# wustl-cig/FLAIR

Measured on AMD Instinct MI355X. Metric: restored frames/sec at 256x256, 16-frame clip, 250-step DDIM, higher is better.
Workload: dtype bf16

## Files before the change

### flair_amd/_lib.py

```python
import ctypes
import os

import torch

_HERE = os.path.dirname(os.path.abspath(__file__))
LIB_PATH = os.path.join(_HERE, "libflair_hip.so")

FLAIR_F32, FLAIR_BF16 = 0, 1
ACT_NONE, ACT_RELU, ACT_LRELU01, ACT_SILU, ACT_DCN_OFFSETS, ACT_LRELU02, ACT_GELU = 0, 1, 2, 3, 4, 5, 6


class FlairHipUnavailable(RuntimeError):
    pass


class FlairHipError(RuntimeError):
    pass


class ConvParams(ctypes.Structure):
    _fields_ = [("dtype", ctypes.c_int), ("T", ctypes.c_int), ("H", ctypes.c_int),
                ("W", ctypes.c_int), ("KT", ctypes.c_int), ("KH", ctypes.c_int),
                ("KW", ctypes.c_int), ("Cout", ctypes.c_int), ("nseg", ctypes.c_int),
                ("seg_c", ctypes.c_int * 4), ("seg_ld", ctypes.c_int * 4),
                ("y_ld", ctypes.c_int), ("res_ld", ctypes.c_int * 2), ("act", ctypes.c_int),
                ("out_scale", ctypes.c_float), ("frame_bias_ld", ctypes.c_int), ("stride", ctypes.c_int),
                ("act_param", ctypes.c_float), ("act_period", ctypes.c_int), ("asym_pad", ctypes.c_int),
                ("reflect_pad", ctypes.c_int)]


_lib = None


def lib():
    global _lib
    if _lib is None:
        global LIB_PATH
        if os.environ.get("FLAIR_HIP_LIB"):
            LIB_PATH = os.environ["FLAIR_HIP_LIB"]
        if not os.path.exists(LIB_PATH):
            raise FlairHipUnavailable(
                f"{LIB_PATH} not found: build it with `python -c 'import __graft_entry__ as g; "
                f"g.build()'` (or `make -C flair_amd/csrc`). The HIP library is required; "
# ... 43 lines not shown
```

### flair_amd/csrc/chain.hip

```cpp
#include <type_traits>

#include "common.h"

namespace {

struct ChainArgs {
    const void* x[4];
    int segC[4], segLd[4], nseg;
    unsigned segBytes[4];
    const void* wA; const float* biasA; int actA; int CinA; unsigned wABytes;
    const void* wB; const float* biasB; int actB; int CoutB; unsigned wBBytes;
    const void* res0; const void* res1; int res0Ld, res1Ld;
    float outScale;
    float actParam; int actPeriod;
    void* y; int yLd;
    int T, H, W;
};

template <typename E> struct MmaC;
template <> struct MmaC<bf16_t> {
    static constexpr int BKE = 32;
    static __device__ __forceinline__ int chunk(int i, int half) { return 2 * i + half; }
    static __device__ __forceinline__ void run(const uint4 (&a)[2], const uint4 (&b)[2], f32x16& acc) {
        acc = __builtin_amdgcn_mfma_f32_32x32x16_bf16(__builtin_bit_cast(bf16x8, a[0]),
                                                      __builtin_bit_cast(bf16x8, b[0]), acc, 0, 0, 0);
        acc = __builtin_amdgcn_mfma_f32_32x32x16_bf16(__builtin_bit_cast(bf16x8, a[1]),
// ... 357 lines not shown
                        }
                    }
                }
            }
        }
        if (batch + 1 < nBatch) {
            write_w(0);
            __syncthreads();
        }
    }
}

struct ResArgs {
    const void* x; int xLd; unsigned xBytes;
    const void* w; unsigned wBytes;
    const float* bias;
    int Cout, act;
    float actParam; int actPeriod;
    float outScale;
    void* y; int yLd;
    int T, H, W;
};

template <int ACT, int NW>
__global__ __launch_bounds__(64 * NW, NW / 4) void conv_resident_kernel(ResArgs a) {
    static_assert(NW == 8, "eight waves of one row");
    prefetch_kernargs<sizeof(ResArgs)>();
    using E = bf16_t;
    constexpr int RPW = 8 / NW;
    constexpr int HWP = 34, HROWS = 10 * HWP, HINSTR = (HROWS + 15) / 16, HBYTES = HINSTR * 1024;
// ... 26 lines not shown
            const int R = k * 16 + lrow;
            const int hr = R / HWP, c = R - hr * HWP;
            const int hh = h0 - 1 + hr, ww = w0 - 1 + c;
            const bool ok = R < HROWS && (unsigned)hh < (unsigned)a.H && (unsigned)ww < (unsigned)a.W;
            const unsigned voff = ok ? (unsigned)(hh * a.W + ww) * ldB + (unsigned)(ch * 64) + (unsigned)((lchunk ^ ((c >> 2) & 3)) << 4) : FLAIR_OOB;
            dma16(xdesc, voff, (unsigned)(ch * HBYTES + k * 1024));
        }
    };
    issue_halo(0);
    unsigned wlane[NWS];
    int wco[NWS];
#pragma unroll
    for (int i = 0; i < NWS; ++i) {
        const int id = (wave * NWS + i) % WINSTR;
        const int row = id * 16 + lrow, tap9 = row >> 6, co = row & 63;
        wlane[i] = (unsigned)((co * 9 + tap9) * 64) * 2u + (unsigned)((lchunk ^ ((co >> 2) & 3)) << 4);
        wco[i] = co;
    }
    auto issue_w = [&](int s_) {
        const int blk = s_ >> 1, ch = s_ & 1;
        const unsigned base = (unsigned)(blk * 64 * 9 * 64) * 2u + (unsigned)(ch * 64);
        const unsigned dst = (unsigned)(RING + (s_ % NRING) * SLOT);
#pragma unroll
        for (int i = 0; i < NWS; ++i) {
            const int id = (wave * NWS + i) % WINSTR;
            dma16(wdesc, blk * 64 + wco[i] < a.Cout ? base + wlane[i] : FLAIR_OOB, dst + (unsigned)(id * 1024));
        }
    };
    auto issue_w_one = [&](int s_, int i) {
        const int blk = s_ >> 1, ch = s_ & 1;
        const unsigned base = (unsigned)(blk * 64 * 9 * 64) * 2u + (unsigned)(ch * 64);
        const int id = (wave * NWS + i) % WINSTR;
        dma16(wdesc, blk * 64 + wco[i] < a.Cout ? base + wlane[i] : FLAIR_OOB, (unsigned)(RING + (s_ % NRING) * SLOT + id * 1024));
    };
    issue_w(0);
    issue_halo(1);
    if (nS > 1) issue_w(1);

    unsigned aoff[2], boff[3][2];
#pragma unroll
    for (int ks = 0; ks < 2; ++ks) {
        aoff[ks] = (unsigned)(lr * 64 + (((2 * ks + lh) ^ ((lr >> 2) & 3)) << 4));
#pragma unroll
        for (int kw = 0; kw < 3; ++kw)
            boff[kw][ks] = (unsigned)((RPW * wave * HWP + kw + lr) * 64 + (((2 * ks + lh) ^ (((kw + lr) >> 2) & 3)) << 4));
    }
// ... 125 lines not shown
        block(blk, acc0, acc1);
        if (blk + 1 < nBlk) block(blk + 1, acc1, acc0);
    }
    if (nBlk & 1) {
#pragma unroll
        for (int g = 0; g < 4 * RPW; ++g) epi_piece(acc0, nBlk - 1, g);
    } else {
#pragma unroll
        for (int g = 0; g < 4 * RPW; ++g) epi_piece(acc1, nBlk - 1, g);
    }
}

int launch_resident(const ChainArgs& c, hipStream_t s) {
    ResArgs a;
    a.x = c.x[0]; a.xLd = c.segLd[0]; a.xBytes = c.segBytes[0];
    a.w = c.wB; a.wBytes = c.wBBytes; a.bias = c.biasB; a.Cout = c.CoutB; a.act = c.actB;
    a.actParam = c.actParam; a.actPeriod = c.actPeriod; a.outScale = c.outScale;
    a.y = c.y; a.yLd = c.yLd; a.T = c.T; a.H = c.H; a.W = c.W;
    constexpr size_t lds = 2 * 22 * 1024 + 3 * 36 * 1024 + 2048;
    const int grid = a.T * (a.H / 8) * (a.W / 32);
    auto go = [&](auto tag) -> int {
        constexpr int ACT = decltype(tag)::value;
        static LdsAttrOnce attr;
        const hipError_t e = flair_max_lds_once(attr, reinterpret_cast<const void*>(&conv_resident_kernel<ACT, 8>));
        FLAIR_CHECK(e == hipSuccess, "flair_conv_chain: hipFuncSetAttribute: %s", hipGetErrorString(e));
        hipLaunchKernelGGL((conv_resident_kernel<ACT, 8>), dim3(grid), dim3(64 * 8), lds, s, a);
        FLAIR_LAUNCH_CHECK();
        return FLAIR_OK;
    };
    if (a.act == FLAIR_ACT_DCN_OFFSETS) return go(std::integral_constant<int, 1>{});
    if (a.act == FLAIR_ACT_SILU) return go(std::integral_constant<int, 2>{});
// ... 367 lines not shown
                "flair_conv_chain: res1 stride/alignment");
    a.res0 = res0; a.res1 = res1; a.res0Ld = p->res_ld[0]; a.res1Ld = p->res_ld[1];
    a.outScale = p->out_scale;
    a.actParam = p->act_param; a.actPeriod = p->act_period;
    FLAIR_CHECK(p->actA != FLAIR_ACT_DCN_OFFSETS && (p->actB != FLAIR_ACT_DCN_OFFSETS ||
                                                       (p->act_period > 0 && p->act_period % 24 == 0)),
                "flair_conv_chain: FLAIR_ACT_DCN_OFFSETS is a stage-B activation with act_period = 3 * deform_groups");
    {
        auto plain = [](int c) { return c == FLAIR_ACT_NONE || c == FLAIR_ACT_RELU || c == FLAIR_ACT_LRELU01 || c == FLAIR_ACT_SILU; };
        FLAIR_CHECK(plain(p->actA) && (plain(p->actB) || p->actB == FLAIR_ACT_DCN_OFFSETS),
                    "flair_conv_chain: activation codes (%d, %d) unsupported: NONE / RELU / LRELU01 / SILU (+ DCN_OFFSETS for stage B)",
                    p->actA, p->actB);
    }
    a.y = y; a.yLd = p->y_ld;
    a.T = p->T; a.H = p->H; a.W = p->W;
    if (!hasA && p->dtype == FLAIR_BF16 && p->C == 64 && p->W % 32 == 0 && p->H % 8 == 0 && !res0 && !res1 &&
        (p->y_ld * 2) % 16 == 0 && p->CoutB % 8 == 0 &&
        (unsigned long long)p->H * p->W * p->y_ld * 2 < 0x40000000ull)
        return launch_resident(a, stream);
    {
        auto lin = [](int c) { return c == FLAIR_ACT_NONE || c == FLAIR_ACT_RELU || c == FLAIR_ACT_LRELU01; };
        if (hasA && p->dtype
 == FLAIR_BF16 && p->C == 64 && p->nseg == 1 && cin == 64 && p->CoutB == 64 && p->W % 32 == 0 &&
            p->H % 8 == 0 && lin(p->actA) && lin(p->actB) && (unsigned long long)p->H * p->W * p->y_ld * 2 < 0x40000000ull &&
            (!res0 || (unsigned long long)p->H * p->W * p->res_ld[0] * 2 < 0x40000000ull) &&
            (!res1 || (unsigned long long)p->H * p->W * p->res_ld[1] * 2 < 0x40000000ull))
            return launch_pair(a, stream);
    }
    if (p->dtype == FLAIR_BF16)
        return hasA ? dispatch_chain<bf16_t, true>(a, p->C, stream) : dispatch_chain<bf16_t, false>(a, p->C, stream);
// ... 3 lines not shown
```

### flair_amd/csrc/conv.hip

```cpp
#include <type_traits>

#include "common.h"

namespace {

struct ConvArgs {
    const void* x[4];
    int segC[4];
    int segLd[4];
    int nseg;
    const void* w;
    const float* bias;
    const void* res0;
    const void* res1;
    int res0Ld, res1Ld;
    void* y;
    int yLd;
    int T, H, W;
    int KT, KH, KW;
    int Cout, CinTot;
    int act;
    float outScale;
    long P;
    int nPixTiles, nCoTiles;
    int tFast;
    unsigned segBytes[4];
    unsigned wBytes;
    float* part;
    int splitK;
    const float* fbias;
    int fbiasLd;
    int stride;
    int tapShift;
    int reflect;
    float actParam;
    int actPeriod;
    int Hin, Win;
    int esz;
};

template <typename E> struct Mma;

template <> struct Mma<bf16_t> {
    static constexpr int BKE = 32;
    static __device__ __forceinline__ int chunk(int i, int half) { return 2 * i + half; }
    static __device__ __forceinline__ void run(const uint4 (&a)[2], const uint4 (&b)[2], f32x16& acc) {
        acc = __builtin_amdgcn_mfma_f32_32x32x16_bf16(__builtin_bit_cast(bf16x8, a[0]),
                                                      __builtin_bit_cast(bf16x8, b[0]), acc, 0, 0, 0);
        acc = __builtin_amdgcn_mfma_f32_32x32x16_bf16(__builtin_bit_cast(bf16x8, a[1]),
                                                      __builtin_bit_cast(bf16x8, b[1]), acc, 0, 0, 0);
    }
    static __device__ __forceinline__ void run1(const uint4& a, const uint4& b, f32x16& acc) {
        acc = __builtin_amdgcn_mfma_f32_32x32x16_bf16(__builtin_bit_cast(bf16x8, a), __builtin_bit_cast(bf16x8, b),
                                                      acc, 0, 0, 0);
// ... 1178 lines not shown
    constexpr int HINSTR = 22, HIMG = HINSTR * 1024, WINSTR = 36, SLOT = WINSTR * 1024;
    constexpr int HR = 3, WR = 2;
    constexpr int RING = HR * HIMG, BIAS = RING + WR * SLOT;
    constexpr int NH = (HINSTR + NW - 1) / NW, NWS = (WINSTR + NW - 1) / NW;
    extern __shared__ __attribute__((aligned(16))) char smem[];
    const int tid = threadIdx.x, lane = tid & 63;
    const int wave = __builtin_amdgcn_readfirstlane(tid >> 6);
    const int lr = lane & 31, lh = lane >> 5;
    const int lrow = lane >> 2, lchunk = lane & 3;
    const int tilesW = a.W / 32, perFrame = tilesW * (a.H / 8);
    const int bid = xcd_remap(blockIdx.x, gridDim.x);
    const int t = bid / perFrame, tile = bid - t * perFrame;
    const int h0 = (tile / tilesW) * 8, w0 = (tile % tilesW) * 32;
    const int nS = a.CinTot / 32;

    const u32x4_t wdesc = make_desc(a.w, a.wBytes);
    const u32x4_t bdesc = make_desc(a.bias, a.bias ? (unsigned)a.Cout * 4u : 0u);
    dma16(bdesc, (unsigned)(lane * 16), (unsigned)BIAS);
    unsigned hpix[NH], hpiece[NH];
#pragma unroll
    for (int i = 0; i < NH; ++i) {
        const int k = (wave * NH + i) % HINSTR;
        const int R = k * 16 + lrow;
        const int hr = R / HWP, c = R - hr * HWP;
        const int hh = h0 - 1 + hr, ww = w0 - 1 + c;
        const bool ok = R < 10 * HWP && (unsigned)hh < (unsigned)a.H && (unsigned)ww < (unsigned)a.W;
        hpix[i] = ok ? (unsigned)(hh * a.W + ww) : 0xffffffffu;
        hpiece[i] = (unsigned)((lchunk ^ ((c >> 2) & 3)) << 4);
    }
    unsigned wlane[NWS];
#pragma unroll
    for (int i = 0; i < NWS; ++i) {
        const int id = (wave * NWS + i) % WINSTR;
        const int row = id * 16 + lrow, tap9 = row >> 6, co = row & 63;
        wlane[i] = co < a.Cout ? (unsigned)((co * 9 + tap9) * a.CinTot) * 2u + (unsigned)((lchunk ^ ((co >> 2) & 3)) << 4) : FLAIR_OOB;
    }
    int hseg = 0, hcb = 0;
    auto issue_halo = [&](int slot) {
        const unsigned ld = (unsigned)a.segLd[hseg] * 2u;
        const u32x4_t xdesc = make_desc(reinterpret_cast<const char*>(a.x[hseg]) + (size_t)t * a.H * a.W * ld, a.segBytes[hseg]);
        const unsigned cofs = (unsigned)(hcb * 64);
#pragma unroll
        for (int i = 0; i < NH; ++i) {
            const int k = (wave * NH + i) % HINSTR;
            dma16(xdesc, hpix[i] == 0xffffffffu ? FLAIR_OOB : hpix[i] * ld + cofs + hpiece[i], (unsigned)(slot * HIMG + k * 1024));
        }
        if (++hcb * 32 >= a.segC[hseg]) {
            hcb = 0;
            ++hseg;
        }
    };
    auto issue_w = [&](int s_) {
#pragma unroll
        for (int i = 0; i < NWS; ++i) {
            const int id = (wave * NWS + i) % WINSTR;
            dma16(wdesc, wlane[i] == FLAIR_OOB ? FLAIR_OOB : wlane[i] + (unsigned)(s_ * 64), (unsigned)(RING + (s_ % WR) * SLOT + id * 1024));
        }
    };
    issue_halo(0);
    issue_w(0);
    if (nS > 1) {
        issue_halo(1);
        issue_w(1);
    }
    if (nS > 2) issue_halo(2);

    unsigned aoff[2], boff[3][2];
#pragma unroll
    for (int ks = 0; ks < 2; ++ks) {
        aoff[ks] = (unsigned)(lr * 64 + (((2 * ks + lh) ^ ((lr >> 2) & 3)) << 4));
#pragma unroll
// ... 431 lines not shown
        return 5;
    }
    const long tiles128 = (long)cdiv(a.P, 128) * cdiv(a.Cout, 128);
    if (a.Cout > 64 && tiles128 >= 512) return 0;
    if (a.Cout >= 128 && a.P >= 1024 && tiles128 <= 64 && (long)a.KT * a.KH * a.KW * a.CinTot >= 2304) return 0;
    const long tiles64x128 = (long)cdiv(a.P, 128) * cdiv(a.Cout, 64);
    if (tiles64x128 >= 512) return 1;
    return 2;
}

template <typename E>
int dispatch(const ConvArgs& a0, hipStream_t s) {
    ConvArgs a = a0;
    const int variant = choose_variant(a);
    a.splitK = a.part ? choose_split(a, variant) : 1;
    switch (variant) {
        case 0: return launch<E, 128, 128, 2, 2>(a, s);
        case 1: return launch<E, 64, 128, 1, 4>(a, s);
        case 2: return launch<E, 64, 64, 2, 2>(a, s);
        case 3: return launch_halo<E, 8, 1, 1>(a, s);
        case 4: return launch_halo<E, 4, 1, 1>(a, s);
        case 6: return launch_halo_ks<E, 8, 1, 2>(a, s);
        case 7: return launch_halo_ks<E, 4, 1, 2>(a, s);
        case 8: return launch_dma<8, 2, 2>(a, s);
        case 9:
            if (frame_kernel_ok(a)) return launch_frame(a, s);
            return launch_dma<8, 1, 2>(a, s);
        default: return launch_halo<E, 2, 1, 1>(a, s);
    }
}
// ... 60 lines not shown
        FLAIR_CHECK(wb < 0x80000000ull, "flair_conv_nhwc: weights span %llu bytes (limit 2 GiB)", wb);
        a.wBytes = (unsigned)wb;
    }
    const int gran = (p->dtype == FLAIR_BF16 && p->Cout % 8 != 0) ? 8 : 16;
    FLAIR_CHECK(p->y_ld >= p->Cout && (p->y_ld * esz) % gran == 0 && ((uintptr_t)y) % 16 == 0,
                "flair_conv_nhwc: output stride/alignment (y_ld = %d: >= Cout = %d, a multiple of %d bytes; y 16-byte aligned)",
                p->y_ld, p->Cout, gran);
    FLAIR_CHECK(!res0 || (p->res_ld[0] >= p->Cout && (p->res_ld[0] * esz) % gran == 0 && ((uintptr_t)res0) % gran == 0),
                "flair_conv_nhwc: res0 stride/alignment (res_ld = %d: >= Cout = %d; stride and pointer multiples of %d bytes)",
                p->res_ld[0], p->Cout, gran);
    FLAIR_CHECK(!res1 || (p->res_ld[1] >= p->Cout && (p->res_ld[1] * esz) % gran == 0 && ((uintptr_t)res1) % gran == 0),
                "flair_conv_nhwc: res1 stride/alignment (res_ld = %d: >= Cout = %d; stride and pointer multiples of %d bytes)",
                p->res_ld[1], p->Cout, gran);
    FLAIR_CHECK(((uintptr_t)w) % 16 == 0, "flair_conv_nhwc: weight alignment");
    FLAIR_CHECK(!bias || ((uintptr_t)bias) % 16 == 0, "flair_conv_nhwc: bias alignment");
    a.nseg = p->nseg;
    a.w = w;
    a.bias = bias;
    a.fbias = frame_bias;
    a.fbiasLd = p->frame_bias_ld;
    FLAIR_CHECK(!frame_bias || p->frame_bias_ld >= p->Cout, "flair_conv_nhwc: frame_bias_ld");
    {
        const unsigned long long hw = (unsigned long long)p->H * p->W * esz;
        FLAIR_CHECK(hw * p->y_ld < 0x40000000ull && (!res0 || hw * p->res_ld[0] < 0x40000000ull) && (!res1 || hw * p->res_ld[1] < 0x40000000ull),
                    "flair_conv_nhwc: one frame of the output / a residual spans more than 1 GiB");
    }
    a.res0 = res0;
    a.res1 = res1;
    a.res0Ld = p->res_ld[0];
    a.res1Ld = p->res_ld[1];
// ... 40 lines not shown
```

### flair_amd/guided_diffusion/packing.py

```python
import torch

from .. import ops


def dev_f32(p, device):
    t = p.detach()
    if t.device != torch.device(device) or t.dtype != torch.float32 or not t.is_contiguous():
        t = t.to(device=device, dtype=torch.float32).contiguous()
    return t


def pack_w(w, dtype, device, segs=None, cout_pad=None):
    w = w.detach().to(device)
    if w.dim() == 2:
        w = w[:, :, None, None]
    cin = w.shape[1]
    return ops.pack_conv_weight(w, segs or [(cin, ops.pad_channels(cin, dtype))], dtype, cout_pad)


def pad_cout(c, g=4):
    return (c + g - 1) // g * g


def pad_bias(b, cpad):
    return torch.cat([b, b.new_zeros(cpad - b.shape[0])]).contiguous()


def fold_bn(conv, bn):
    w = conv.weight.detach().float()
    b = conv.bias.detach().float() if conv.bias is not None else w.new_zeros(w.shape[0])
    if bn is not None:
        g = bn.weight.detach().float() / torch.sqrt(bn.running_var.detach().float() + bn.eps)
# ... 65 lines not shown
```

### flair_amd/guided_diffusion/unet_new.py

```python
import math

import torch
import torch.nn as nn

from .. import ops
from .nn_new import conv_nd, linear, normalization, zero_module
from .packing import PackedModel, dev_f32, pack_w, packed_conv, pk_int, run_conv

A = ops


class PlaceHolder(nn.Module):

    def __init__(self, module):
        super().__init__()
        self.wrapped_module = module


LazyReshaper2D = LazyReshaper3D = PlaceHolder


class TemporalWrapper(PlaceHolder):
    """unet_new.py:50-59 (skipped when ``enable_cross_frames`` is False)."""

# ... 214 lines not shown
        super().__init__()
        self.conv1 = nn.Conv2d(mid_channels, mid_channels, 3, 1, 1, bias=True)
        self.conv2 = nn.Conv2d(mid_channels, mid_channels, 3, 1, 1, bias=True)


class ResidualBlocksWithInputConv(nn.Module):

    def __init__(self, in_channels, out_channels=64, num_blocks=1):
        super().__init__()
        if num_blocks != 1:
            raise NotImplementedError("flair_amd: FLAIR uses one residual block per trunk")
        self.main = nn.Sequential(nn.Conv2d(in_channels, out_channels, 3, 1, 1, bias=True),
                                  nn.LeakyReLU(negative_slope=0.1),
                                  nn.Sequential(ResidualBlockNoBN(out_channels)))

    def pack(self, dtype, device, split):
        c = self.main[0].out_channels
        rb = self.main[2][0]
        return dict(w0=pack_w(self.main[0].weight, dtype, device, [(s, s) for s in split]),
                    b0=dev_f32(self.main[0].bias, device),
                    w1=pack_w(rb.conv1.weight, dtype, device, [(c, c)]), b1=dev_f32(rb.conv1.bias, device),
                    w2=pack_w(rb.conv2.weight, dtype, device, [(c, c)]), b2=dev_f32(rb.conv2.bias, device))




def run_trunk(pk, segs, c, *, extra_res=None, out=None, out_scale=1.0):
    k = (1, 3, 3)
    t1 = ops.conv(segs, pk["w0"], pk["b0"], c, k, act=A.ACT_LRELU01)
    if c == 64 and ops.chain_supported(t1, c):
        return ops.conv_chain(t1, pk["w1"], pk["b1"], A.ACT_RELU, pk["w2"], pk["b2"], A.ACT_NONE, c, c,
                              res0=t1, res1=extra_res, out=out, out_scale=out_scale)
    t2 = ops.conv(t1, pk["w1"], pk["b1"], c, k, act=A.ACT_RELU)
    return ops.conv(t2, pk["w2"], pk["b2"], c, k, res0=t1, res1=extra_res, out=out, out_scale=out_scale)


class SecondOrderDeformableAlignment(nn.Module):

    def __init__(self, in_channels, out_channels, kernel_size=3, padding=1, deform_groups=16,
                 max_residue_magnitude=10):
        super().__init__()
        assert kernel_size == 3 and padding == 1
        self.in_channels, self.out_channels = in_channels, out_channels
        self.deform_groups, self.max_residue_magnitude = deform_groups, max_residue_magnitude
# ... 4 lines not shown
            self.weight.uniform_(-stdv, stdv)
        c = out_channels
        self.conv_offset = nn.Sequential(
            nn.Conv2d(3 * c + 4, c, 3, 1, 1), nn.LeakyReLU(negative_slope=0.1),
            nn.Conv2d(c, c, 3, 1, 1), nn.LeakyReLU(negative_slope=0.1),
            nn.Conv2d(c, c, 3, 1, 1), nn.LeakyReLU(negative_slope=0.1),
            nn.Conv2d(c, 27 * deform_groups, 3, 1, 1))
        zero_module(self.conv_offset[-1])

    def pack(self, dtype, device):
        c = self.out_channels
        ka = ops.k_align(dtype)
        co = self.conv_offset
        perm = ops.dcn_raw_permutation(self.deform_groups)
        w6, b6 = co[6].weight.detach()[perm], co[6].bias.detach()[perm]
        return dict(
            w0=pack_w(co[0].weight, dtype, device, [(c, c), (c, c), (c, c), (4, ka)]), b0=dev_f32(co[0].bias, device),
            w2=pack_w(co[2].weight, dtype, device, [(c, c)]), b2=dev_f32(co[2].bias, device),
            w4=pack_w(co[4].weight, dtype, device, [(c, c)]), b4=dev_f32(co[4].bias, device),
            w6=pack_w(w6, dtype, device, [(c, c)]), b6=dev_f32(b6, device),
            wd=pack_w(self.weight, dtype, device, [(2 * c, 2 * c)]), bd=dev_f32(self.bias, device))


class BasicVSRPP(nn.Module):

    def __init__(self, mid_channels=64, max_residue_magnitude=10, use_checkpoint=False):
        super().__init__()
        self.mid_channels = mid_channels
        self.deform_align = nn.ModuleDict()
        self.backbone = nn.ModuleDict()
        for i, name in enumerate(["backward_1", "forward_1"]):
            self.deform_align[name] = SecondOrderDeformableAlignment(
                2 * mid_channels, mid_channels, 3, padding=1, deform_groups=16,
                max_residue_magnitude=max_residue_magnitude)
            self.backbone[name] = ResidualBlocksWithInputConv((2 + i) * mid_channels, mid_channels, 1)
        self.reconstruction = ResidualBlocksWithInputConv(3 * mid_channels, mid_channels, 1)
        self.conv_last = zero_module(nn.Conv2d(mid_channels, mid_channels, 1, 1))

    def pack(self, dtype, device):
        c = self.mid_channels
        self._pk = dict(
            align={n: m.pack(dtype, device) for n, m in self.deform_align.items()},
            trunk={"backward_1": self.backbone["backward_1"].pack(dtype, device, [c, c]),
                   "forward_1": self.backbone["forward_1"].pack(dtype, device, [c, c, c])},
            recon=self.reconstruction.pack(dtype, device, [c, c, c]),
            wl=pack_w(self.conv_last.weight, dtype, device, [(c, c)]), bl=dev_f32(self.conv_last.bias, device))

    def _propagate(self, ctx, hidden, flows, name, others, weight, wmaps, dest):
        pk_a, pk_t = self._pk["align"][name], self._pk["trunk"][name]
        T, H, W, c = hidden.shape
        order = list(range(T))
        flow_idx = list(range(-1, T - 1))
        if "backward" in name:
            order = order[::-1]
            flow_idx = order
        zero_c = torch.zeros((1, H, W, c), dtype=ctx.dtype, device=ctx.device)
        ka = ops.k_align(ctx.dtype)
        k3 = (1, 3, 3)
        G = self.deform_align[name].deform_groups
# ... 10 lines not shown
                cond_n1 = torch.empty_like(zero_c)
                second = i > 1
                feat_n2 = prev2 if second else zero_c
                cond_n2 = torch.empty_like(zero_c) if second else zero_c
                if cached is not None:
                    flow_n2, flowpad = cached[i - 1]
                    ops.vsrpp_warp2(prop, feat_n2 if second else None, flow_n1, flow_n2, cond_n1, cond_n2 if second else None)
                else:
                    flowpad = torch.zeros((1, H, W, ka), dtype=ctx.dtype, device=ctx.device)
                    flow_n2 = torch.empty_like(flow_n1) if second else None
                    ops.vsrpp_prep(prop, feat_n2 if second else None, flow_n1,
                                   flows[flow_idx[i - 1]:flow_idx[i - 1] + 1] if second else None,
                                   cond_n1, cond_n2 if second else None, flow_n2, flowpad)
                    if fill is not None:
                        fill.append((flow_n2, flowpad))
                o = ops.conv([cond_n1, cur, cond_n2, flowpad], pk_a["w0"], pk_a["b0"], c, k3, act=A.ACT_LRELU01)
                if c == 64 and ops.chain_supported(o, c):
                    o = ops.conv_chain(o, pk_a["w2"], pk_a["b2"], A.ACT_LRELU01, pk_a["w4"], pk_a["b4"],
                                       A.ACT_LRELU01, c, c)
                else:
                    o = ops.conv(o, pk_a["w2"], pk_a["b2"], c, k3, act=A.ACT_LRELU01)
                    o = ops.conv(o, pk_a["w4"], pk_a["b4"], c, k3, act=A.ACT_LRELU01)
                if c == 64 and ops.chain_supported(o, c) and W % 32 == 0:
                    raw = ops.conv_chain(o, None, None, A.ACT_NONE, pk_a["w6"], pk_a["b6"], A.ACT_DCN_OFFSETS, c, 27 * G,
                                         act_param=mag, act_period=3 * G)
                else:
                    raw = ops.conv(o, pk_a["w6"], pk_a["b6"], 27 * G, k3, act=A.ACT_DCN_OFFSETS, act_param=mag,
                                   act_period=3 * G)
                aligned = ops.dcn_align(prop, feat_n2, raw, flow_n1, flow_n2, pk_a["wd"], pk_a["bd"], c,
                                        groups=G, max_mag=mag, raw_activated=True)

            else:
                aligned = zero_c
            segs = [cur] + [o_[idx:idx + 1] for o_ in others] + [aligned]
            new = run_trunk(pk_t, segs, c, extra_res=aligned, out=dest[idx:idx + 1], out_scale=weight)
            if wmaps is not None:
                ops.scale_pixels(new, wmaps[idx])
            prev2, prop = (prop if i > 0 else None), new
        if fill is not None:
            store[key] = fill
# ... 373 lines not shown
```

### flair_amd/ops.py

```python
import ctypes

import torch

from . import _lib
from ._lib import (ACT_DCN_OFFSETS, ACT_GELU, ACT_LRELU01, ACT_LRELU02, ACT_NONE, ACT_RELU, ACT_SILU, ConvParams, check, dtype_code, lib,
                   ptr, stream)

__all__ = ["conv", "conv_chain", "group_norm", "nchw_to_clip", "clip_to_nchw", "timestep_embedding", "linear",
           "qkv_attention", "temporal_attention", "flow_warp", "flow_compose", "resize",
           "dcn_align", "dcn_raw_permutation", "scale_pixels", "predict_xstart", "sampler_update",
           "ACT_NONE", "ACT_RELU", "ACT_LRELU01", "ACT_SILU", "ACT_DCN_OFFSETS", "ACT_LRELU02", "ACT_GELU"]


class GnParams(ctypes.Structure):
    _fields_ = [("dtype", ctypes.c_int), ("C", ctypes.c_int), ("c0", ctypes.c_int),
                ("ld0", ctypes.c_int), ("ld1", ctypes.c_int), ("groups", ctypes.c_int),
                ("F", ctypes.c_int), ("H", ctypes.c_int), ("W", ctypes.c_int),
                ("frames_per_stat", ctypes.c_int), ("eps", ctypes.c_float), ("act", ctypes.c_int),
                ("resample", ctypes.c_int), ("y_ld", ctypes.c_int), ("raw_ld", ctypes.c_int),
                ("film_ld", ctypes.c_int)]


class SamplerCoefs(ctypes.Structure):
    _fields_ = [("gamma", ctypes.c_float), ("w_aux", ctypes.c_float),
# ... 39 lines not shown
def _f32(t):
    assert t is None or (t.dtype == torch.float32 and t.is_contiguous())
    return t


def k_align(dtype):
    return 32 if dtype == torch.bfloat16 else 16


def pad_channels(c, dtype):
    g = k_align(dtype)
    return (c + g - 1) // g * g


def conv(xs, weight, bias, cout, kernel, *, out=None, act=ACT_NONE, res0=None, res1=None,
         out_scale=1.0, stride=1, frame_bias=None, act_param=0.0, act_period=0, asym_pad=False, reflect_pad=False):
    if isinstance(xs, torch.Tensor):
        xs = [xs]
    x0 = xs[0]
    T, H, W, _ = x0.shape
    p = ConvParams()
    p.dtype = dtype_code(x0)
    p.T, p.H, p.W = T, H, W
    p.KT, p.KH, p.KW = kernel
    p.Cout = cout
    p.nseg = len(xs)
    arr = (ctypes.c_void_p * 4)()
    for i, x in enumerate(xs):
        assert x.dtype == x0.dtype and x.shape[:3] == x0.shape[:3]
        p.seg_c[i] = x.shape[3]
        p.seg_ld[i] = _ld(x)
# ... 3 lines not shown
    p.reflect_pad = int(reflect_pad)
    p.frame_bias_ld = frame_bias.stride(0) if frame_bias is not None else 0
    if frame_bias is not None:
        assert frame_bias.dtype == torch.float32 and frame_bias.stride(1) == 1 and frame_bias.shape[0] == T
    Ho, Wo = (H + stride - 1) // stride, (W + stride - 1) // stride
    if out is None:
        out = torch.empty((T, Ho, Wo, cout), dtype=x0.dtype, device=x0.device)
    assert tuple(out.shape[:3]) == (T, Ho, Wo) and out.shape[3] >= cout and out.dtype == x0.dtype
    p.y_ld = _ld(out)
    p.res_ld[0] = _ld(res0) if res0 is not None else 0
    p.res_ld[1] = _ld(res1) if res1 is not None else 0
    p.act = act
    p.act_param, p.act_period = act_param, act_period
    p.out_scale = out_scale
    assert weight.dtype == x0.dtype and weight.is_contiguous()
    e0 = _prof_begin()
    wsb = _conv_ws_bytes(p)
    ws = _workspace(wsb, x0.device, "conv") if wsb else None

    def launch(_keep=xs):
        check(lib().flair_conv_nhwc(ctypes.byref(p), arr, ptr(weight), ptr(_f32(bias)), ptr(frame_bias), ptr(res0),
                                    ptr(res1), ptr(out), ptr(ws), ctypes.c_size_t(wsb), stream()), "flair_conv_nhwc")
    launch()
    if e0 is not None:
        cin = sum(x.shape[3] for x in xs)
        taps = kernel[0] * kernel[1] * kernel[2]
        esz = x0.element_size()
        flops = 2.0 * T * Ho * Wo * cout * cin * taps
        nbytes = esz * (cin * T * H * W + cout * T * Ho * Wo * (1 + (res0 is not None) + (res1 is not None))
                        + cout * taps * cin)
        _prof_end(e0, ("conv", lib().flair_conv_variant(ctypes.byref(p))), x0.dtype, flops, nbytes, launch,
                  ("conv", T, H, W, tuple(x.shape[3] for x in xs), cout, tuple(kernel), stride, act,
                   res0 is not None, res1 is not None, frame_bias is not None))
    return out

# ... 44 lines not shown
    w = w.reshape(cout, cin, taps).permute(0, 2, 1).float()
    parts, o = [], 0
    for real, padded in seg_channels:
        seg = w[:, :, o:o + real]
        if padded > real:
            seg = torch.cat([seg, seg.new_zeros(cout, taps, padded - real)], dim=2)
        parts.append(seg)
        o += real
    assert o == cin, (o, cin)
    w = torch.cat(parts, dim=2)
    if cout_pad is not None and cout_pad > cout:
        w = torch.cat([w, w.new_zeros(cout_pad - cout, taps, w.shape[2])], dim=0)
    return w.to(dtype).contiguous()


class ChainParams(ctypes.Structure):
    _fields_ = [("dtype", ctypes.c_int), ("T", ctypes.c_int), ("H", ctypes.c_int), ("W", ctypes.c_int),
                ("C", ctypes.c_int), ("CoutB", ctypes.c_int), ("nseg", ctypes.c_int),
                ("seg_c", ctypes.c_int * 4), ("seg_ld", ctypes.c_int * 4), ("y_ld", ctypes.c_int),
                ("res_ld", ctypes.c_int * 2), ("actA", ctypes.c_int), ("actB", ctypes.c_int),
                ("out_scale", ctypes.c_float), ("act_param", ctypes.c_float), ("act_period", ctypes.c_int)]


def chain_supported(xs, c_mid):
    x0 = xs[0] if isinstance(xs, (list, tuple)) else xs
    T, H, W, _ = x0.shape
    tiles = T * ((H + 7) // 8) * (W // 32 if W % 32 == 0 and T * ((H + 7) // 8) * (W // 32) >= 192 else W // 8)
    return c_mid in (64, 128) and W % 8 == 0 and tiles <= 512


def conv_chain(xs, wA, bA, actA, wB, bB, actB, c_mid, coutB, *, res0=None, res1=None, out_scale=1.0, out=None,
               act_param=0.0, act_period=0):
    if isinstance(xs, torch.Tensor):
        xs = [xs]
    x0 = xs[0]
    T, H, W, _ = x0.shape
    p = ChainParams()
    p.dtype = dtype_code(x0)
    p.T, p.H, p.W = T, H, W
    p.C, p.CoutB = c_mid, coutB
    p.nseg = len(xs)
    arr = (ctypes.c_void_p * 4)()
    for i, x in enumerate(xs):
        assert x.dtype == x0.dtype and x.shape[:3] == x0.shape[:3]
        p.seg_c[i] = x.shape[3]
        p.seg_ld[i] = _ld(x)
        arr[i] = x.data_ptr()
    if out is None:
        out = torch.empty((T, H, W, coutB), dtype=x0.dtype, device=x0.device)
    assert tuple(out.shape[:3]) == (T, H, W) and out.shape[3] >= coutB and out.dtype == x0.dtype
    p.y_ld = _ld(out)
    p.res_ld[0] = _ld(res0) if res0 is not None else 0
    p.res_ld[1] = _ld(res1) if res1 is not None else 0
    p.actA, p.actB = actA, actB
    p.act_param, p.act_period = act_param, act_period
    p.out_scale = out_scale
    assert wB.dtype == x0.dtype and wB.is_contiguous() and (wA is None or (wA.dtype == x0.dtype and wA.is_contiguous()))
    e0 = _prof_begin()

    def launch(_keep=xs):
        check(lib().flair_conv_chain(ctypes.byref(p), arr, ptr(wA), ptr(_f32(bA)), ptr(wB), ptr(_f32(bB)), ptr(res0),
                                     ptr(res1), ptr(out), stream()), "flair_conv_chain")
    launch()
    if e0 is not None:
        cin = sum(x.shape[3] for x in xs)
        esz = x0.element_size()
        px = T * H * W
        flops = 2.0 * 9 * px * (c_mid * coutB + (cin * c_mid if wA is not None else 0))
        nbytes = esz * (px * (cin + coutB * (1 + (res0 is not None) + (res1 is not None)))
                        + 9 * c_mid * coutB + (9 * cin * c_mid if wA is not None else 0))
        _prof_end(e0, ("chain", 2 if wA is not None else 1, c_mid), x0.dtype, flops, nbytes, launch,
                  ("chain", T, H, W, tuple(x.shape[3] for x in xs), c_mid, coutB, wA is not None, res0 is not None,
                   res1 is not None))
    return out

# ... 942 lines not shown
```

### include/flair_hip.h

```cpp
#ifndef FLAIR_HIP_H
#define FLAIR_HIP_H

#include <stddef.h>
#include <stdint.h>

#ifdef __cplusplus
extern "C" {
#endif

#ifndef __HIP_PLATFORM_AMD__
typedef struct ihipStream_t* hipStream_t;
#endif

typedef enum {
    FLAIR_OK = 0,
    FLAIR_ERR_ARG = -1,
    FLAIR_ERR_HIP = -2
} flair_status;

typedef enum { FLAIR_F32 = 0, FLAIR_BF16 = 1 } flair_dtype;

typedef enum {
    FLAIR_ACT_NONE = 0,
    FLAIR_ACT_RELU = 1,
// ... 13 lines not shown
    int KT, KH, KW;
    int Cout;
    int nseg;
    int seg_c[4];
    int seg_ld[4];
    int y_ld;
    int res_ld[2];
    int act;
    float out_scale;
    int frame_bias_ld;
    int stride;
    float act_param;
    int act_period;
    int asym_pad;
    int reflect_pad;
} flair_conv_params;

size_t flair_conv_workspace_bytes(const flair_conv_params* p);
int flair_conv_nhwc(const flair_conv_params* p, const void* const* x, const void* w,
                    const float* bias, const float* frame_bias, const void* res0, const void* res1,
                    void* y, void* workspace, size_t workspace_bytes, hipStream_t stream);
int flair_conv_variant(const flair_conv_params* p);


typedef struct {
    int dtype;
    int T, H, W;
    int C;
    int CoutB;
    int nseg;
    int seg_c[4];
    int seg_ld[4];
    int y_ld;
    int res_ld[2];
    int actA, actB;
    float out_scale;
    float act_param;
    int act_period;
} flair_chain_params;

int flair_conv_chain(const flair_chain_params* p, const void* const* x, const void* wA, const float* biasA,
                     const void* wB, const float* biasB, const void* res0, const void* res1, void* y,
                     hipStream_t stream);


typedef struct {
    int dtype;
    int C, c0;
    int ld0, ld1;
    int groups;
    int F, H, W;
    int frames_per_stat;
    float eps;
// ... 212 lines not shown
```

Baseline: 0.8541.

## Add chunk-major weight images for frame and resident conv kernels

Adds an optional pre-packed chunk-major weight layout (kt, cin/32, cout-block, 9, 64, 32) so that each 32-channel input stage of the weights is a contiguous block. The frame conv kernel (variant 9) and the resident chain kernel then fetch weights with contiguous per-stage addressing instead of strided per-row reads across the full Cin. The packed copies are built once at model pack time for the BasicVSR++ trunk and deform-align convolutions. The cost is extra weight memory and more struct and ABI fields; other kernel variants ignore the new pointer.

```diff
diff --git a/flair_amd/_lib.py b/flair_amd/_lib.py
--- a/flair_amd/_lib.py
+++ b/flair_amd/_lib.py
@@ -26,7 +26,7 @@
                 ("y_ld", ctypes.c_int), ("res_ld", ctypes.c_int * 2), ("act", ctypes.c_int),
                 ("out_scale", ctypes.c_float), ("frame_bias_ld", ctypes.c_int), ("stride", ctypes.c_int),
                 ("act_param", ctypes.c_float), ("act_period", ctypes.c_int), ("asym_pad", ctypes.c_int),
-                ("reflect_pad", ctypes.c_int)]
+                ("reflect_pad", ctypes.c_int), ("w_cm", ctypes.c_void_p)]
 
 
 _lib = None
diff --git a/flair_amd/csrc/chain.hip b/flair_amd/csrc/chain.hip
--- a/flair_amd/csrc/chain.hip
+++ b/flair_amd/csrc/chain.hip
@@ -10,6 +10,7 @@
     unsigned segBytes[4];
     const void* wA; const float* biasA; int actA; int CinA; unsigned wABytes;
     const void* wB; const float* biasB; int actB; int CoutB; unsigned wBBytes;
+    const void* wBcm;
     const void* res0; const void* res1; int res0Ld, res1Ld;
     float outScale;
     float actParam; int actPeriod;
@@ -397,6 +398,7 @@
 struct ResArgs {
     const void* x; int xLd; unsigned xBytes;
     const void* w; unsigned wBytes;
+    int cm;
     const float* bias;
     int Cout, act;
     float actParam; int actPeriod;
@@ -453,12 +455,15 @@
     for (int i = 0; i < NWS; ++i) {
         const int id = (wave * NWS + i) % WINSTR;
         const int row = id * 16 + lrow, tap9 = row >> 6, co = row & 63;
-        wlane[i] = (unsigned)((co * 9 + tap9) * 64) * 2u + (unsigned)((lchunk ^ ((co >> 2) & 3)) << 4);
+        wlane[i] = (a.cm ? (unsigned)row * 64u : (unsigned)((co * 9 + tap9) * 64) * 2u) + (unsigned)((lchunk ^ ((co >> 2) & 3)) << 4);
         wco[i] = co;
     }
+    auto stage_base = [&](int blk, int ch) {
+        return a.cm ? (unsigned)(ch * nBlk + blk) * (9u * 64u * 64u) : (unsigned)(blk * 64 * 9 * 64) * 2u + (unsigned)(ch * 64);
+    };
     auto issue_w = [&](int s_) {
         const int blk = s_ >> 1, ch = s_ & 1;
-        const unsigned base = (unsigned)(blk * 64 * 9 * 64) * 2u + (unsigned)(ch * 64);
+        const unsigned base = stage_base(blk, ch);
         const unsigned dst = (unsigned)(RING + (s_ % NRING) * SLOT);
 #pragma unroll
         for (int i = 0; i < NWS; ++i) {
@@ -468,7 +473,7 @@
     };
     auto issue_w_one = [&](int s_, int i) {
         const int blk = s_ >> 1, ch = s_ & 1;
-        const unsigned base = (unsigned)(blk * 64 * 9 * 64) * 2u + (unsigned)(ch * 64);
+        const unsigned base = stage_base(blk, ch);
         const int id = (wave * NWS + i) % WINSTR;
         dma16(wdesc, blk * 64 + wco[i] < a.Cout ? base + wlane[i] : FLAIR_OOB, (unsigned)(RING + (s_ % NRING) * SLOT + id * 1024));
     };
@@ -624,7 +629,10 @@
 int launch_resident(const ChainArgs& c, hipStream_t s) {
     ResArgs a;
     a.x = c.x[0]; a.xLd = c.segLd[0]; a.xBytes = c.segBytes[0];
-    a.w = c.wB; a.wBytes = c.wBBytes; a.bias = c.biasB; a.Cout = c.CoutB; a.act = c.actB;
+    a.cm = c.wBcm != nullptr;
+    a.w = a.cm ? c.wBcm : c.wB;
+    a.wBytes = a.cm ? 2u * (unsigned)cdiv(c.CoutB, 64) * (9u * 64u * 64u) : c.wBBytes;
+    a.bias = c.biasB; a.Cout = c.CoutB; a.act = c.actB;
     a.actParam = c.actParam; a.actPeriod = c.actPeriod; a.outScale = c.outScale;
     a.y = c.y; a.yLd = c.yLd; a.T = c.T; a.H = c.H; a.W = c.W;
     constexpr size_t lds = 2 * 22 * 1024 + 3 * 36 * 1024 + 2048;
@@ -1022,6 +1030,10 @@
     }
     a.y = y; a.yLd = p->y_ld;
     a.T = p->T; a.H = p->H; a.W = p->W;
+    if (p->dtype == FLAIR_BF16 && p->wB_cm) {
+        FLAIR_CHECK(((uintptr_t)p->wB_cm) % 128 == 0, "flair_conv_chain: wB_cm must be 128-byte aligned");
+        a.wBcm = p->wB_cm;
+    }
     if (!hasA && p->dtype == FLAIR_BF16 && p->C == 64 && p->W % 32 == 0 && p->H % 8 == 0 && !res0 && !res1 &&
         (p->y_ld * 2) % 16 == 0 && p->CoutB % 8 == 0 &&
         (unsigned long long)p->H * p->W * p->y_ld * 2 < 0x40000000ull)
diff --git a/flair_amd/csrc/conv.hip b/flair_amd/csrc/conv.hip
--- a/flair_amd/csrc/conv.hip
+++ b/flair_amd/csrc/conv.hip
@@ -37,7 +37,11 @@
     int actPeriod;
     int Hin, Win;
     int esz;
+    const void* wcm;
+    unsigned wcmBytes;
 };
+
+constexpr unsigned WCM_STAGE_BYTES = 9 * 64 * 64;
 
 template <typename E> struct Mma;
 
@@ -1246,7 +1250,9 @@
     const int h0 = (tile / tilesW) * 8, w0 = (tile % tilesW) * 32;
     const int nS = a.CinTot / 32;
 
-    const u32x4_t wdesc = make_desc(a.w, a.wBytes);
+    const bool cm = a.wcm != nullptr;
+    const u32x4_t wdesc = cm ? make_desc(a.wcm, a.wcmBytes) : make_desc(a.w, a.wBytes);
+    const unsigned wstep = cm ? WCM_STAGE_BYTES : 64u;
     const u32x4_t bdesc = make_desc(a.bias, a.bias ? (unsigned)a.Cout * 4u : 0u);
     dma16(bdesc, (unsigned)(lane * 16), (unsigned)BIAS);
     unsigned hpix[NH], hpiece[NH];
@@ -1265,7 +1271,7 @@
     for (int i = 0; i < NWS; ++i) {
         const int id = (wave * NWS + i) % WINSTR;
         const int row = id * 16 + lrow, tap9 = row >> 6, co = row & 63;
-        wlane[i] = co < a.Cout ? (unsigned)((co * 9 + tap9) * a.CinTot) * 2u + (unsigned)((lchunk ^ ((co >> 2) & 3)) << 4) : FLAIR_OOB;
+        wlane[i] = co < a.Cout ? (cm ? (unsigned)row * 64u : (unsigned)((co * 9 + tap9) * a.CinTot) * 2u) + (unsigned)((lchunk ^ ((co >> 2) & 3)) << 4) : FLAIR_OOB;
     }
     int hseg = 0, hcb = 0;
     auto issue_halo = [&](int slot) {
@@ -1286,7 +1292,7 @@
 #pragma unroll
         for (int i = 0; i < NWS; ++i) {
             const int id = (wave * NWS + i) % WINSTR;
-            dma16(wdesc, wlane[i] == FLAIR_OOB ? FLAIR_OOB : wlane[i] + (unsigned)(s_ * 64), (unsigned)(RING + (s_ % WR) * SLOT + id * 1024));
+            dma16(wdesc, wlane[i] == FLAIR_OOB ? FLAIR_OOB : wlane[i] + (unsigned)s_ * wstep, (unsigned)(RING + (s_ % WR) * SLOT + id * 1024));
         }
     };
     issue_halo(0);
@@ -1748,6 +1754,7 @@
     ConvArgs a = a0;
     const int variant = choose_variant(a);
     a.splitK = a.part ? choose_split(a, variant) : 1;
+    if (!(variant == 9 && frame_kernel_ok(a))) a.wcm = nullptr;
     switch (variant) {
         case 0: return launch<E, 128, 128, 2, 2>(a, s);
         case 1: return launch<E, 64, 128, 1, 4>(a, s);
@@ -1838,6 +1845,13 @@
                 p->res_ld[1], p->Cout, gran);
     FLAIR_CHECK(((uintptr_t)w) % 16 == 0, "flair_conv_nhwc: weight alignment");
     FLAIR_CHECK(!bias || ((uintptr_t)bias) % 16 == 0, "flair_conv_nhwc: bias alignment");
+    if (p->w_cm && p->dtype == FLAIR_BF16 && p->KH == 3 && p->KW == 3) {
+        const unsigned long long cb = (unsigned long long)p->KT * (a.CinTot / 32) * ((p->Cout + 63) / 64) * WCM_STAGE_BYTES;
+        FLAIR_CHECK(cb < 0x80000000ull, "flair_conv_nhwc: chunk-major weight image spans %llu bytes (limit 2 GiB)", cb);
+        FLAIR_CHECK(((uintptr_t)p->w_cm) % 128 == 0, "flair_conv_nhwc: w_cm must be 128-byte aligned");
+        a.wcm = p->w_cm;
+        a.wcmBytes = (unsigned)cb;
+    }
     a.nseg = p->nseg;
     a.w = w;
     a.bias = bias;
diff --git a/flair_amd/guided_diffusion/packing.py b/flair_amd/guided_diffusion/packing.py
--- a/flair_amd/guided_diffusion/packing.py
+++ b/flair_amd/guided_diffusion/packing.py
@@ -16,6 +16,13 @@
         w = w[:, :, None, None]
     cin = w.shape[1]
     return ops.pack_conv_weight(w, segs or [(cin, ops.pad_channels(cin, dtype))], dtype, cout_pad)
+
+
+def add_cm(pk, *names):
+    for n in names:
+        if pk[n].dtype == torch.bfloat16:
+            pk[n + "_cm"] = ops.pack_conv_weight_cm(pk[n], pk[n].shape[1] // 9)
+    return pk
 
 
 def pad_cout(c, g=4):
diff --git a/flair_amd/guided_diffusion/unet_new.py b/flair_amd/guided_diffusion/unet_new.py
--- a/flair_amd/guided_diffusion/unet_new.py
+++ b/flair_amd/guided_diffusion/unet_new.py
@@ -5,7 +5,7 @@
 
 from .. import ops
 from .nn_new import conv_nd, linear, normalization, zero_module
-from .packing import PackedModel, dev_f32, pack_w, packed_conv, pk_int, run_conv
+from .packing import PackedModel, add_cm, dev_f32, pack_w, packed_conv, pk_int, run_conv
 
 A = ops
 
@@ -252,20 +252,21 @@
                                   nn.LeakyReLU(negative_slope=0.1),
                                   nn.Sequential(ResidualBlockNoBN(out_channels)))
 
-    def pack(self, dtype, device, split):
+    def pack(self, dtype, device, split, per_frame=False):
         c = self.main[0].out_channels
         rb = self.main[2][0]
-        return dict(w0=pack_w(self.main[0].weight, dtype, device, [(s, s) for s in split]),
-                    b0=dev_f32(self.main[0].bias, device),
-                    w1=pack_w(rb.conv1.weight, dtype, device, [(c, c)]), b1=dev_f32(rb.conv1.bias, device),
-                    w2=pack_w(rb.conv2.weight, dtype, device, [(c, c)]), b2=dev_f32(rb.conv2.bias, device))
+        pk = dict(w0=pack_w(self.main[0].weight, dtype, device, [(s, s) for s in split]),
+                  b0=dev_f32(self.main[0].bias, device),
+                  w1=pack_w(rb.conv1.weight, dtype, device, [(c, c)]), b1=dev_f32(rb.conv1.bias, device),
+                  w2=pack_w(rb.conv2.weight, dtype, device, [(c, c)]), b2=dev_f32(rb.conv2.bias, device))
+        return add_cm(pk, "w0") if per_frame and c == 64 else pk
 
 
 
 
 def run_trunk(pk, segs, c, *, extra_res=None, out=None, out_scale=1.0):
     k = (1, 3, 3)
-    t1 = ops.conv(segs, pk["w0"], pk["b0"], c, k, act=A.ACT_LRELU01)
+    t1 = ops.conv(segs, pk["w0"], pk["b0"], c, k, act=A.ACT_LRELU01, w_cm=pk.get("w0_cm"))
     if c == 64 and ops.chain_supported(t1, c):
         return ops.conv_chain(t1, pk["w1"], pk["b1"], A.ACT_RELU, pk["w2"], pk["b2"], A.ACT_NONE, c, c,
                               res0=t1, res1=extra_res, out=out, out_scale=out_scale)
@@ -300,12 +301,13 @@
         co = self.conv_offset
         perm = ops.dcn_raw_permutation(self.deform_groups)
         w6, b6 = co[6].weight.detach()[perm], co[6].bias.detach()[perm]
-        return dict(
+        pk = dict(
             w0=pack_w(co[0].weight, dtype, device, [(c, c), (c, c), (c, c), (4, ka)]), b0=dev_f32(co[0].bias, device),
             w2=pack_w(co[2].weight, dtype, device, [(c, c)]), b2=dev_f32(co[2].bias, device),
             w4=pack_w(co[4].weight, dtype, device, [(c, c)]), b4=dev_f32(co[4].bias, device),
             w6=pack_w(w6, dtype, device, [(c, c)]), b6=dev_f32(b6, device),
             wd=pack_w(self.weight, dtype, device, [(2 * c, 2 * c)]), bd=dev_f32(self.bias, device))
+        return add_cm(pk, "w0", "w6") if c == 64 else pk
 
 
 class BasicVSRPP(nn.Module):
@@ -327,8 +329,8 @@
         c = self.mid_channels
         self._pk = dict(
             align={n: m.pack(dtype, device) for n, m in self.deform_align.items()},
-            trunk={"backward_1": self.backbone["backward_1"].pack(dtype, device, [c, c]),
-                   "forward_1": self.backbone["forward_1"].pack(dtype, device, [c, c, c])},
+            trunk={"backward_1": self.backbone["backward_1"].pack(dtype, device, [c, c], per_frame=True),
+                   "forward_1": self.backbone["forward_1"].pack(dtype, device, [c, c, c], per_frame=True)},
             recon=self.reconstruction.pack(dtype, device, [c, c, c]),
             wl=pack_w(self.conv_last.weight, dtype, device, [(c, c)]), bl=dev_f32(self.conv_last.bias, device))
 
@@ -369,7 +371,8 @@
                                    cond_n1, cond_n2 if second else None, flow_n2, flowpad)
                     if fill is not None:
                         fill.append((flow_n2, flowpad))
-                o = ops.conv([cond_n1, cur, cond_n2, flowpad], pk_a["w0"], pk_a["b0"], c, k3, act=A.ACT_LRELU01)
+                o = ops.conv([cond_n1, cur, cond_n2, flowpad], pk_a["w0"], pk_a["b0"], c, k3, act=A.ACT_LRELU01,
+                             w_cm=pk_a.get("w0_cm"))
                 if c == 64 and ops.chain_supported(o, c):
                     o = ops.conv_chain(o, pk_a["w2"], pk_a["b2"], A.ACT_LRELU01, pk_a["w4"], pk_a["b4"],
                                        A.ACT_LRELU01, c, c)
@@ -378,7 +381,7 @@
                     o = ops.conv(o, pk_a["w4"], pk_a["b4"], c, k3, act=A.ACT_LRELU01)
                 if c == 64 and ops.chain_supported(o, c) and W % 32 == 0:
                     raw = ops.conv_chain(o, None, None, A.ACT_NONE, pk_a["w6"], pk_a["b6"], A.ACT_DCN_OFFSETS, c, 27 * G,
-                                         act_param=mag, act_period=3 * G)
+                                         act_param=mag, act_period=3 * G, wB_cm=pk_a.get("w6_cm"))
                 else:
                     raw = ops.conv(o, pk_a["w6"], pk_a["b6"], 27 * G, k3, act=A.ACT_DCN_OFFSETS, act_param=mag,
                                    act_period=3 * G)
diff --git a/flair_amd/ops.py b/flair_amd/ops.py
--- a/flair_amd/ops.py
+++ b/flair_amd/ops.py
@@ -77,7 +77,8 @@
 
 
 def conv(xs, weight, bias, cout, kernel, *, out=None, act=ACT_NONE, res0=None, res1=None,
-         out_scale=1.0, stride=1, frame_bias=None, act_param=0.0, act_period=0, asym_pad=False, reflect_pad=False):
+         out_scale=1.0, stride=1, frame_bias=None, act_param=0.0, act_period=0, asym_pad=False, reflect_pad=False,
+         w_cm=None):
     if isinstance(xs, torch.Tensor):
         xs = [xs]
     x0 = xs[0]
@@ -111,11 +112,15 @@
     p.act_param, p.act_period = act_param, act_period
     p.out_scale = out_scale
     assert weight.dtype == x0.dtype and weight.is_contiguous()
+    if w_cm is not None:
+        assert w_cm.dtype == x0.dtype == torch.bfloat16 and w_cm.is_contiguous() and tuple(kernel[1:]) == (3, 3) and \
+            tuple(w_cm.shape) == weight_cm_shape(cout, kernel[0], sum(x.shape[3] for x in xs)), tuple(w_cm.shape)
+        p.w_cm = w_cm.data_ptr()
     e0 = _prof_begin()
     wsb = _conv_ws_bytes(p)
     ws = _workspace(wsb, x0.device, "conv") if wsb else None
 
-    def launch(_keep=xs):
+    def launch(_keep=(xs, w_cm)):
         check(lib().flair_conv_nhwc(ctypes.byref(p), arr, ptr(weight), ptr(_f32(bias)), ptr(frame_bias), ptr(res0),
                                     ptr(res1), ptr(out), ptr(ws), ctypes.c_size_t(wsb), stream()), "flair_conv_nhwc")
     launch()
@@ -190,12 +195,31 @@
     return w.to(dtype).contiguous()
 
 
+def weight_cm_shape(cout, kt, cin):
+    return (kt, cin // 32, (cout + 63) // 64, 9, 64, 32)
+
+
+def pack_conv_weight_cm(wp, kt=1):
+    cout, taps, cin = wp.shape
+    assert wp.dtype == torch.bfloat16 and taps == kt * 9 and cin % 32 == 0, (wp.dtype, tuple(wp.shape), kt)
+    nb = (cout + 63) // 64
+    if nb * 64 > cout:
+        wp = torch.cat([wp, wp.new_zeros(nb * 64 - cout, taps, cin)], dim=0)
+    return wp.reshape(nb, 64, kt, 9, cin // 32, 32).permute(2, 4, 0, 3, 1, 5).contiguous()
+
+
+def unpack_conv_weight_cm(img, cout):
+    kt, nch, nb = img.shape[:3]
+    return img.permute(2, 4, 0, 3, 1, 5).reshape(nb * 64, kt * 9, nch * 32)[:cout].contiguous()
+
+
 class ChainParams(ctypes.Structure):
     _fields_ = [("dtype", ctypes.c_int), ("T", ctypes.c_int), ("H", ctypes.c_int), ("W", ctypes.c_int),
                 ("C", ctypes.c_int), ("CoutB", ctypes.c_int), ("nseg", ctypes.c_int),
                 ("seg_c", ctypes.c_int * 4), ("seg_ld", ctypes.c_int * 4), ("y_ld", ctypes.c_int),
                 ("res_ld", ctypes.c_int * 2), ("actA", ctypes.c_int), ("actB", ctypes.c_int),
-                ("out_scale", ctypes.c_float), ("act_param", ctypes.c_float), ("act_period", ctypes.c_int)]
+                ("out_scale", ctypes.c_float), ("act_param", ctypes.c_float), ("act_period", ctypes.c_int),
+                ("wB_cm", ctypes.c_void_p)]
 
 
 def chain_supported(xs, c_mid):
@@ -206,7 +230,7 @@
 
 
 def conv_chain(xs, wA, bA, actA, wB, bB, actB, c_mid, coutB, *, res0=None, res1=None, out_scale=1.0, out=None,
-               act_param=0.0, act_period=0):
+               act_param=0.0, act_period=0, wB_cm=None):
     if isinstance(xs, torch.Tensor):
         xs = [xs]
     x0 = xs[0]
@@ -232,9 +256,13 @@
     p.act_param, p.act_period = act_param, act_period
     p.out_scale = out_scale
     assert wB.dtype == x0.dtype and wB.is_contiguous() and (wA is None or (wA.dtype == x0.dtype and wA.is_contiguous()))
+    if wB_cm is not None:
+        assert wB_cm.dtype == x0.dtype == torch.bfloat16 and wB_cm.is_contiguous() and \
+            tuple(wB_cm.shape) == weight_cm_shape(coutB, 1, c_mid), tuple(wB_cm.shape)
+        p.wB_cm = wB_cm.data_ptr()
     e0 = _prof_begin()
 
-    def launch(_keep=xs):
+    def launch(_keep=(xs, wB_cm)):
         check(lib().flair_conv_chain(ctypes.byref(p), arr, ptr(wA), ptr(_f32(bA)), ptr(wB), ptr(_f32(bB)), ptr(res0),
                                      ptr(res1), ptr(out), stream()), "flair_conv_chain")
     launch()
diff --git a/include/flair_hip.h b/include/flair_hip.h
--- a/include/flair_hip.h
+++ b/include/flair_hip.h
@@ -51,6 +51,7 @@
     int act_period;
     int asym_pad;
     int reflect_pad;
+    const void* w_cm;
 } flair_conv_params;
 
 size_t flair_conv_workspace_bytes(const flair_conv_params* p);
@@ -74,6 +75,7 @@
     float out_scale;
     float act_param;
     int act_period;
+    const void* wB_cm;
 } flair_chain_params;
 
 int flair_conv_chain(const flair_chain_params* p, const void* const* x, const void* wA, const float* biasA,
```

Result: no change. 0.8583, median of 6 (+0.5%).
